# Computational-Genomics-BSC/GenomeAnonymizer

Measured on AMD Instinct MI355X. Metric: reads/sec + bases/sec anonymized, 150 bp paired BAM, 1/2/4/8 MI355X, higher is better.
Workload: dtype u8

## Files before the change

genomeanonymizer_amd/csrc/ganon_batch.h:

```cpp
#ifndef GANON_BATCH_H
#define GANON_BATCH_H

#include <hip/hip_runtime.h>

#include <cstdint>
#include <vector>

#include "../../include/ganon.h"
#include "ganon_ctx.h"

namespace ganon_dev {

constexpr int kBlock = 256;
constexpr int kWaves = kBlock / 64;
constexpr int kTile = 16384;

enum { kSkipClassify = 1, kSkipChunks = 2, kSkipCopy = 4, kSkipCounts = 8 };
constexpr int kGrpRec = 5;
constexpr int kGrpObs = 512;
constexpr int kGrpMaxScopes = 256;
constexpr int kGrpMaxSpan = 1 << 20;
constexpr int64_t kPartAlign = 128;
constexpr int kSegMaxLen = (1 << 14) - 1;
constexpr uint32_t kSegMine = 1u << 31;
// ... 174 lines not shown
  ganon_ref *own_ref = nullptr;
  ganon_dev::DBuf b_ref_start, b_read_len, b_seq_off, b_cig_off, b_n_cig, b_dataset, b_write_scope, b_seq, b_cigar,
      b_incid_off, b_incid_read, b_span_start, b_span_len, b_ref_off, b_keep_pos, b_keep_code;
  ganon_dev::DBuf b_part;
  ganon_dev::DBuf b_long;
  ganon_dev::DBuf b_nseg, b_scost, b_scan_tmp, b_slots, b_slot0;
  ganon_dev::DBuf b_wspart;
  ganon_dev::DBuf b_order;
  int64_t max_scope_incid = 0;
  bool ordered = false;
  ganon_dev::DBuf b_read_end, b_cursor, b_gs0, b_lo, b_linemap, b_groups, b_seg4, b_grp_part, b_far, b_gokey, b_gopay, b_gtkey, b_gtflag, b_out,
      b_scope_calls, b_scope_bases, b_small;
  uint8_t *out = nullptr;
  int32_t *scope_calls = nullptr, *scope_bases = nullptr;
  unsigned long long *totals = nullptr, *static_totals = nullptr, *acc = nullptr, *far_count = nullptr;
  int32_t *rare_tiles = nullptr;
  int32_t *status = nullptr;
  unsigned int *long_count = nullptr;
  unsigned long long *far_need = nullptr;
  size_t flags_bytes = 0;
  ganon_dev::PrepErr *err = nullptr;
  unsigned long long *plan_info = nullptr;
  unsigned long long *paths = nullptr;
  unsigned long long *gated = nullptr;
  unsigned long long *cursor = nullptr;
  ganon_dev::GrpAux *aux = nullptr;
  int32_t n_groups = 0, group_target = 512;
  bool spec = false, spec_ready = false;
  bool spec_sized = false;
  int64_t spec_sizes[4] = {-1, -1, -1, -1};
  bool long_mode = false;
  bool flat_mode = false;
  bool fused = false;
  ganon_dev::DBuf b_desc, b_cand, b_sdirty;
  ganon_dev::DBuf b_xrec, b_xlist, b_xcnt, b_xidx;
  int64_t xcap = 0;
  unsigned int *xcount = nullptr;
  ganon_dev::DBuf b_inc4, b_rbase, b_rrec;
  int64_t n_rrec = 0, n_long_seg = 0;
  unsigned long long *cand = nullptr;
  int64_t *scost = nullptr;
  int64_t n_seg = 0, region = 0, far_cap = 0, n_written = 0, region_per_incid = 0, n_id_ops = 0;
  int64_t max_len = 0, max_seg = 0;
  int64_t far_cap_alloc = 0;
  std::vector<unsigned long long> cursor_h;
  ganon_dev::GrpAux aux_h{};
  unsigned long long static_h[GANON_N_TOTALS] = {0};
  std::vector<void *> huge_allocs;
  ganon_dev::Tile *tiles_h = nullptr;
  int32_t *large_incid = nullptr, *large_written_h = nullptr, *large_ids = nullptr;
  int64_t *tab_off = nullptr;
  uint16_t *tn_tab = nullptr;
  int64_t tn_entries = 0;
  int32_t n_tiles_h = 0, n_large_written_h = 0, n_huge_scopes = 0;
  int32_t *rare_tile_list = nullptr;
  bool ran = false;
};

namespace ganon_prep {

int plan(ganon_ctx *ctx, ganon_dbatch *db, bool allow_spec);
int run(ganon_ctx *ctx, ganon_dbatch *db);
int ws_diag(ganon_ctx *ctx, ganon_dbatch *db);
int batch_error(ganon_ctx *ctx, ganon_dbatch *db);
int grow(ganon_ctx *ctx, ganon_dev::DBuf &b, size_t bytes);
template <typename T>
inline int grow_n(ganon_ctx *ctx, ganon_dev::DBuf &b, size_t count, T **out) {
  int rc = grow(ctx, b, count * sizeof(T));
  *out = static_cast<T *>(b.p);
  return rc;
}

}
// ... 21 lines not shown
```

genomeanonymizer_amd/csrc/ganon_hip.hip:

```cpp
#include <hip/hip_runtime.h>
#include <map>
#include <mutex>

#include <algorithm>
#include <cstdarg>
#include <cstdio>
#include <cstring>
#include <numeric>
#include <string>
#include <type_traits>
#include <vector>

#include "../../include/ganon.h"
#include "ganon_batch.h"
#include "ganon_ctx.h"

using namespace ganon_dev;

namespace {

__global__ void __launch_bounds__(kBlock) k_ref2(const uint8_t *__restrict__ ref, int64_t n_words,
                                                 uint32_t *__restrict__ ref2) {
  for (int64_t w = blockIdx.x * (int64_t)kBlock + threadIdx.x; w < n_words; w += (int64_t)gridDim.x * kBlock) {
    const uint64_t v = load16(ref, 16 * w);
// ... 91 lines not shown
    atomicMax(far_need, n_far_all);
  }
}
}

using ganon_detail::check_launch;
using ganon_detail::fail;
using ganon_detail::KernelScope;

namespace {

constexpr int64_t kFarMaxEntries = int64_t(1) << 30;

void free_buf(DBuf &b) {
  if (b.p) hipFree(b.p);
  b = DBuf{};
}

void free_ref(ganon_ref *r) {
  if (!r) return;
  if (r->nt16) hipFree(r->nt16);
  if (r->ref2) hipFree(r->ref2);
  if (r->bad) hipFree(r->bad);
  delete r;
}

void free_batch(ganon_dbatch *db) {
  DBuf *bufs[] = {&db->b_ref_start, &db->b_read_len, &db->b_seq_off, &db->b_cig_off, &db->b_n_cig, &db->b_dataset,
                  &db->b_write_scope, &db->b_seq, &db->b_cigar, &db->b_incid_off, &db->b_incid_read,
                  &db->b_span_start, &db->b_span_len, &db->b_ref_off, &db->b_keep_pos, &db->b_keep_code,
                  &db->b_read_end, &db->b_wspart, &db->b_cursor, &db->b_gs0, &db->b_lo, &db->b_linemap, &db->b_groups,
                  &db->b_seg4, &db->b_grp_part, &db->b_far, &db->b_gokey, &db->b_gopay, &db->b_gtkey, &db->b_gtflag,
                  &db->b_out, &db->b_scope_calls, &db->b_scope_bases, &db->b_small, &db->b_part, &db->b_long, &db->b_nseg,
                  &db->b_scost, &db->b_scan_tmp, &db->b_slots, &db->b_slot0, &db->b_order, &db->b_desc, &db->b_cand,
                  &db->b_sdirty, &db->b_inc4, &db->b_rbase, &db->b_rrec, &db->b_xrec, &db->b_xlist, &db->b_xcnt, &db->b_xidx};
  for (DBuf *b : bufs) free_buf(*b);
  ganon_huge::release(db);
  free_ref(db->own_ref);
  db->own_ref = nullptr;
}

template <typename T>
int h2d(ganon_ctx *ctx, DBuf &b, const T *src, size_t count, const T **field) {
  T *p = nullptr;
  int rc = ganon_prep::grow_n(ctx, b, count, &p);
  if (rc) return rc;
  if (count) {
    hipError_t e = hipMemcpyAsync(p, src, count * sizeof(T), hipMemcpyHostToDevice, ctx->stream);
    if (e != hipSuccess) return fail(ctx, GANON_E_DEVICE, "hipMemcpyAsync H2D failed: %s", hipGetErrorString(e));
  }
  *field = p;
  return GANON_OK;
}

int ref_create(ganon_ctx *ctx, const uint8_t *nt16, int64_t bytes, ganon_ref **out) {
  *out = nullptr;
  if (bytes < 0 || (bytes > 0 && !nt16)) return fail(ctx, GANON_E_ARG, "bad reference buffer");
  if (2 * bytes >= (int64_t(1) << 40)) return fail(ctx, GANON_E_ARG, "reference over 2^40 bases");
  ganon_ref *r = new ganon_ref();
  r->bytes = bytes;
  r->n_blk = (bytes + 31) / 32;
  const int64_t n_words = (2 * bytes + 15) / 16;
  const int64_t n_bad = (r->n_blk + 63) / 64 + 1;
  hipError_t e = hipMalloc(reinterpret_cast<void **>(&r->nt16), (size_t)bytes + 128);
  if (e == hipSuccess) e = hipMalloc(reinterpret_cast<void **>(&r->ref2), (size_t)(n_words + 2) * 4 + 128);
  if (e == hipSuccess) e = hipMalloc(reinterpret_cast<void **>(&r->bad), (size_t)n_bad * 8 + 128);
  if (e != hipSuccess) {
// ... 767 lines not shown
```

genomeanonymizer_amd/csrc/ganon_prep.hip:

```cpp
#include <hip/hip_runtime.h>

#include <algorithm>
#include <cstring>
#include <type_traits>

#include <rocprim/device/device_scan.hpp>


#include "ganon_batch.h"

using namespace ganon_dev;
using ganon_detail::check_launch;
using ganon_detail::fail;
using ganon_detail::KernelScope;

namespace {

constexpr int kPrepThreads = 256;
constexpr unsigned long long kNone = ~0ull;
constexpr int kCursors = 256;
constexpr int64_t kFarMax = int64_t(1) << 28;

struct Raw {
  const int32_t *ref_start, *read_len, *n_cig, *write_scope;
// ... 33 lines not shown
  return cost ? cost[s] / target : (incid_off[s] + weight * s) / target;
}

enum { kPartWritten = 0, kPartMaxLen, kPartMaxSeg, kPartIdOps, kPartHuge, kPartWsHash, kParts };

__device__ __forceinline__ unsigned long long block_sum_u64(unsigned long long v, unsigned long long *ws) {
  for (int o = 32; o > 0; o >>= 1) {
    const uint32_t lo = __shfl_xor((uint32_t)v, o), hi = __shfl_xor((uint32_t)(v >> 32), o);
    v += ((unsigned long long)hi << 32) | lo;
  }
  __syncthreads();
  if ((threadIdx.x & 63) == 0) ws[threadIdx.x >> 6] = v;
  __syncthreads();
  unsigned long long t = 0;
  for (int w = 0; w < kWaves; ++w) t += ws[w];
  return t;
}
#ifndef GANON_SCAN_U
#define GANON_SCAN_U 4
#endif
constexpr int kScanReadsPerBlock = GANON_SCAN_U * kPrepThreads;
constexpr int kScanScopesPerBlock = 4 * kPrepThreads;

struct ScanOut {
  int32_t *read_end;
  int32_t *long_list;
  unsigned int *long_count;
  longlong2 *gmeta;
  int64_t g_bound;
  unsigned long long *part;
  int64_t part_stride;
  int32_t *nseg;
  int4 *desc;
  unsigned long long *cand;
  int32_t *xidx;
  int4 *xrec;
  unsigned int *xcount;
  uint32_t xper;
};


__device__ __forceinline__ unsigned long long shfl64(unsigned long long v, int lane) {
  const uint32_t lo = __shfl((uint32_t)v, lane), hi = __shfl((uint32_t)(v >> 32), lane);
  return ((unsigned long long)hi << 32) | lo;
}

__device__ __forceinline__ void scan_candidate(unsigned long long *__restrict__ cand, long long key, int64_t so) {
  const unsigned long long v = ~(unsigned long long)so;
  const int lane = threadIdx.x & 63;
  unsigned long long pending = __ballot(key >= 0);
  while (pending) {
    const int leader = __ffsll((long long)pending) - 1;
    const uint32_t klo = __builtin_amdgcn_readlane((uint32_t)key, leader),
                   khi = __builtin_amdgcn_readlane((uint32_t)((unsigned long long)key >> 32), leader);
    const long long lk = (long long)(((unsigned long long)khi << 32) | klo);
    const bool same = key == lk;
    unsigned long long x = same ? v : 0ull;
#pragma unroll
    for (int o = 32; o > 0; o >>= 1) {
      const unsigned long long y = shfl64(x, lane ^ o);
      x = y > x ? y : x;
    }
    if (lane == leader) atomicMax(&cand[lk], x);
    pending &= ~__ballot(same);
  }
}

__device__ __forceinline__ void block_parts(unsigned long long (&acc)[kParts], unsigned long long *__restrict__ part,
                                            int64_t stride) {
  __shared__ unsigned long long ws[kWaves][kParts];
  const int lane = threadIdx.x & 63, wave = threadIdx.x >> 6;
#pragma unroll
  for (int k = 0; k < kParts; ++k) {
    unsigned long long v = acc[k];
#pragma unroll
    for (int o = 32; o > 0; o >>= 1) {
      const unsigned long long x = shfl64(v, lane ^ o);
      v = (k == kPartMaxLen || k == kPartMaxSeg) ? (x > v ? x : v) : v + x;
    }
    if (lane == 0) ws[wave][k] = v;
  }
  __syncthreads();
  if (threadIdx.x < kParts) {
    const int k = threadIdx.x;
    unsigned long long v = 0;
    for (int w = 0; w < kWaves; ++w)
      v = (k == kPartMaxLen || k == kPartMaxSeg) ? (ws[w][k] > v ? ws[w][k] : v) : v + ws[w][k];
    part[stride * k + blockIdx.x] = v;
  }
}

struct CigarWalk {
  long long rl;
  int ns, nid, bad_op;
};

__device__ __forceinline__ CigarWalk wave_cigar_walk(const uint32_t *__restrict__ cg, int nc, int L) {
  const int lane = threadIdx.x & 63;
// ... 55 lines not shown
    int L[kScanU], nc[kScanU], rs[kScanU], ws[kScanU], ds[kScanU];
    Off co[kScanU], so[kScanU];
    bool ok[kScanU];
    {
      int64_t co64[kScanU], so64[kScanU];
#pragma unroll
      for (int u = 0; u < kScanU; ++u) {
        const int64_t r = r0 + tid + kPrepThreads * u;
        ok[u] = r < r1;
        const int64_t rr = ok[u] ? r : r0;
        L[u] = R.read_len[rr];
        nc[u] = R.n_cig[rr];
        co64[u] = R.cig_off[rr];
        rs[u] = R.ref_start[rr];
        so64[u] = R.seq_off[rr];
        ws[u] = R.write_scope[rr];
        ds[u] = R.dataset[rr];
      }
#pragma unroll
      for (int u = 0; u < kScanU; ++u) {
        const int64_t r = r0 + tid + kPrepThreads * u;
        if (ok[u]) {
          if (L[u] < 0 || so64[u] < 0 || so64[u] + ((int64_t)L[u] + 1) / 2 > R.seq_bytes) { report(err, kErrReadSeq, r); ok[u] = false; }
          else if (nc[u] < 0 || co64[u] < 0 || co64[u] + nc[u] > R.n_cigar_ops) { report(err, kErrReadCigar, r); ok[u] = false; }
          if (ds[u] > 1) report(err, kErrReadDataset, r);
          if (ws[u] < -1 || ws[u] >= R.n_scopes) { report(err, kErrReadWriteScope, r, ws[u]); ok[u] = false; }
          if (L[u] >= (1 << 24)) report(err, kErrReadLong, r);
        }
        co[u] = ok[u] ? (Off)co64[u] : (Off)0;
        so[u] = ok[u] ? (Off)so64[u] : (Off)0;
      }
    }
    uint32_t w0[kScanU];
    int wo[kScanU];
#pragma unroll
    for (int u = 0; u < kScanU; ++u) {
      w0[u] = ok[u] && nc[u] > 0 ? R.cigar[co[u]] : 0u;
      wo[u] = O.cand && ok[u] && ws[u] >= 0 && L[u] > 0 ? (int)R.incid_off[ws[u]] : -1;
    }
    if (O.cand) {
#pragma unroll
      for (int u = 0; u < kScanU; ++u) {
        long long key = -1;
        if (wo[u] >= 0) {
          const uint64_t x = (uint64_t)wo[u] + (uint64_t)weight * (uint64_t)ws[u];
          int64_t g = x >> 32 ? (int64_t)(x / (uint64_t)target) : (int64_t)((uint32_t)x / (uint32_t)target);
          g = g < 0 ? 0 : (g > O.g_bound - 1 ? O.g_bound - 1 : g);
          key = 2 * g + (ds[u] & 1);
        }
        scan_candidate(O.cand, key, (int64_t)so[u]);
      }
    }
#pragma unroll
    for (int u = 0; u < kScanU; ++u) {
      const int64_t r = r0 + tid + kPrepThreads * u;
      if (ok[u]) {
        n_wr += ws[u] >= 0;
        if (ws[u] >= 0) hsum += ws_hash((int)r);
        mx_len = max(mx_len, (uint32_t)L[u]);
        if (nc[u] > kScanLongCigar) {
          O.long_list[atomicAdd(O.long_count, 1u)] = (int32_t)r;
          continue;
        }
        int64_t rl = 0;
        int q = 0, ns = 0, nid = 0;
        int fq = 0, fn = 0;
        int fp = 0;
        bool good = true;
        for (int k = 0; k < nc[u]; ++k) {
          const uint32_t w = k == 0 ? w0[u] : R.cigar[co[u] + k];
          const int op = (int)(w & 0xF);
          const int len = (int)(w >> 4);
          if (op > 8) { report(err, kErrCigarOp, r, op); good = false; break; }
          if (is_aligned_op(op)) {
            if (q < L[u]) {
              if (ns == 0) {
                fq = q;
                fp = (int)rl;
                fn = min(min(len, L[u] - q), kSegMaxLen);
              }
              ns += (min(len, L[u] - q) + kSegMaxLen - 1) / kSegMaxLen;
            }
            q += len;
            rl += len;
          } else if (op == 1 || op == 4) {
// ... 388 lines not shown

__global__ void __launch_bounds__(kPrepThreads) k_prep_pieces(const unsigned long long *__restrict__ lo, int n_cand,
                                                              LineMap M, int64_t seq_bytes, int4 *__restrict__ groups,
                                                              const unsigned long long *__restrict__ gate) {
  if (gate) {
    if (gate[7]) return;
    n_cand = (int)min((unsigned long long)n_cand, 2 * gate[5]);
  }
  for (int64_t c = blockIdx.x * (int64_t)kPrepThreads + threadIdx.x; c < n_cand; c += (int64_t)gridDim.x * kPrepThreads) {
    const unsigned long long k = lo[c];
    int4 pc = piece(0, 0);
    if (k != kNone) {
      const int64_t line = (int64_t)(k >> 7);
      unsigned long long win = 0;
      for (unsigned h = hash_line(line, M.hsize);; h = (h + 1) & (unsigned)(M.hsize - 1))
        if (M.hkey[h] == (unsigned long long)line + 1) {
          win = M.hval[h];
          break;
        }
      if ((win & ((1ull << 25) - 1)) == (unsigned long long)c) {
        const int64_t next = map_next(M, line);
        const int64_t a = map_any_below(M, line) ? line * kPartAlign : 0;
        pc = piece(a, next < 0 ? seq_bytes : next * kPartAlign);
      }
    } else if (c == 0) {
      bool any = false;
      for (int64_t w = 0; w < M.n2 && !any; ++w) any = M.l2[w] != 0;
      if (!any) pc = piece(0, seq_bytes);
    }
    groups[kGrpRec * (c >> 1) + 2 + 2 * (c & 1)] = pc;
  }
}

__global__ void __launch_bounds__(kPrepThreads) k_prep_cands(const Raw R, const longlong2 *__restrict__ gmeta,
                                                             int n_groups, long long region_per_incid,
                                                             const unsigned long long *__restrict__ cand,
                                                             unsigned long long *__restrict__ lo, int4 *__restrict__ groups,
                                                             LineMap M, unsigned long long *__restrict__ ws_part,
                                                             const unsigned long long *__restrict__ gate,
                                                             uint8_t *__restrict__ sdirty, const uint64_t *__restrict__ bad,
                                                             int64_t n_blk) {
  const int64_t g = blockIdx.x * (int64_t)kPrepThreads + threadIdx.x;
  if (gate[7]) return;
  if (g < R.n_scopes) {
    const int64_t sl = R.span_len[g], ro = R.ref_off[g];
    sdirty[g] = sl > 0 && sl <= kGrpMaxSpan && !ref_clean(bad, n_blk, ro, (int)sl);
  }
  if (g >= n_groups) return;
  if ((unsigned long long)g >= gate[5]) {
    ws_part[g] = 0;
    return;
  }
  const longlong2 m0 = gmeta[g];
  const longlong2 m1 = (unsigned long long)g + 1 < gate[5] ? gmeta[g + 1] : make_longlong2(R.n_scopes, R.n_incid);
  const int s0 = (int)m0.x, s1 = (int)m1.x;
  const int64_t i0 = m0.y, i1 = m1.y;
  const int64_t region = i0 * region_per_incid + (int64_t)kGrpObs * g;
  const int cap = (int)min((i1 - i0) * region_per_incid + kGrpObs, (long long)(INT32_MAX / 2));
  groups[kGrpRec * g] = make_int4(s0, s1, (int)(uint32_t)i0, (int)(uint32_t)((uint64_t)i0 >> 32));
  groups[kGrpRec * g + 1] = make_int4((int)(uint32_t)i1, (int)(uint32_t)((uint64_t)i1 >> 32), (int)(uint32_t)i1,
                                      (int)(uint32_t)((uint64_t)i1 >> 32));
  groups[kGrpRec * g + 3] = make_int4((int)(uint32_t)region, (int)(uint32_t)((uint64_t)region >> 32), cap, 0);
#pragma unroll
  for (int d = 0; d < 2; ++d) {
    const unsigned long long c = cand[2 * g + d];
    const unsigned long long k = c ? ~c : kNone;
    lo[2 * g + d] = k;
    if (k != kNone) map_mark(M, k, (uint32_t)(2 * g + d));
  }
}

__device__ __forceinline__ void block_scan2(int a, int b, int &ea, int &eb, int &ta, int &tb, int *ws) {
  const int lane = threadIdx.x & 63, wave = threadIdx.x >> 6;
  int ia = a, ib = b;
#pragma unroll
  for (int o = 1; o < 64; o <<= 1) {
    const int xa = __shfl_up(ia, o), xb = __shfl_up(ib, o);
    if (lane >= o) {
      ia += xa;
      ib += xb;
    }
  }
  if (lane == 63) {
    ws[wave] = ia;
    ws[kWaves + wave] = ib;
  }
  __syncthreads();
  int ba = 0, bb = 0;
  ta = tb = 0;
#pragma unroll
  for (int w = 0; w < kWaves; ++w) {
    const int va = ws[w], vb = ws[kWaves + w];
    if (w < wave) {
      ba += va;
      bb += vb;
    }
    ta += va;
    tb += vb;
  }
  ea = ba + ia - a;
  eb = bb + ib - b;
  __syncthreads();
// ... 791 lines not shown
    return rc;
  db->B.read_end = read_end;
  db->ran = false;
  const Raw R = raw_of(db);
  const int tgt0 = ctx->group_target ? ctx->group_target : 704;
  const long long w0 = weight_of(tgt0);
  const int64_t g_bound = ns ? (db->n_incid + w0 * (ns - 1)) / tgt0 + 1 : 1;
  const bool want_fused = ctx->fused_flat && (ctx->prep_long == -1 || ctx->prep_long == 2);
  const bool same = db->spec_ready && db->spec_sizes[0] == nr && db->spec_sizes[1] == ns &&
                    db->spec_sizes[2] == db->n_incid && db->spec_sizes[3] == tgt0 && db->flat_mode &&
                    ctx->last_plan == db && db->fused == want_fused;
  ctx->last_plan = db;
  const bool sized = !same && ctx->spec_shape_ok && ctx->spec_tgt == tgt0 && ctx->prep_long == -1;
  const bool spec = allow_spec && ctx->spec_plan && (same || sized);
  db->spec = spec;
  db->spec_sized = spec && sized;
  if (!spec) {
    db->n_groups = 0;
    db->spec_ready = false;
  }
  db->fused = want_fused;
  const int64_t spec_rpi = !spec ? 0 : db->spec_sized ? ctx->spec_rpi : db->region_per_incid;
  longlong2 *gm = nullptr;
  unsigned long long *part = nullptr;
  const int64_t rb = (nr + kScanReadsPerBlock - 1) / kScanReadsPerBlock;
  const int64_t sb = (ns + kScanScopesPerBlock - 1) / kScanScopesPerBlock;
  const int64_t nb = std::max<int64_t>(1, rb + sb);
  if (nb > INT32_MAX) return fail(ctx, GANON_E_ARG, "batch too large");
  int32_t *long_list = nullptr;
  if ((rc = grow_n(ctx, db->b_gs0, (size_t)g_bound, &gm)) ||
      (rc = grow_n(ctx, db->b_part, (size_t)kParts * (nb + kLongGrid), &part)) ||
      (rc = grow_n(ctx, db->b_long, (size_t)std::max<int64_t>(nr, 1), &long_list)))
    return rc;
  unsigned long long *cand = nullptr;
  int4 *desc = nullptr, *xrec = nullptr;
  int2 *xlist = nullptr;
  int32_t *xidx = nullptr;
  uint8_t *sdirty = nullptr;
  if (db->fused) {
    const int64_t xwant = std::min<int64_t>(
        INT32_MAX, ctx->xrec_init > 0 && db->xcap == 0 ? (int64_t)ctx->xrec_init
                                                       : std::max<int64_t>({db->xcap, int64_t(65536), nr / 8}));
    if ((rc = grow_n(ctx, db->b_desc, (size_t)std::max<int64_t>(nr, 1), &desc)) ||
        (rc = grow_n(ctx, db->b_cand, 2 * (size_t)g_bound, &cand)) ||
        (rc = grow_n(ctx, db->b_sdirty, (size_t)std::max<int64_t>(ns, 1), &sdirty)) ||
        (rc = grow_n(ctx, db->b_xrec, (size_t)xwant, &xrec)) ||
        (rc = grow_n(ctx, db->b_xlist, (size_t)std::max<int64_t>(db->n_incid, 1), &xlist)) ||
        (rc = grow_n(ctx, db->b_xidx, (size_t)std::max<int64_t>(nr, 1), &xidx)))
      return rc;
    db->xcap = std::min<int64_t>(INT32_MAX, (int64_t)((db->b_xrec.bytes - 128) / sizeof(int4)));
    if (ctx->xrec_init > 0 && db->xcap > xwant) db->xcap = xwant;
  }
  db->cand = cand;
  unsigned int *long_count = db->long_count;
  const int64_t pstride = nb + kLongGrid;
  if ((rc = grow_n(ctx, db->b_xcnt, (size_t)kXStripes * kXStride, &db->xcount))) return rc;
  const ScanOut O{read_end, long_list, long_count, gm, g_bound, part, pstride, nullptr, desc, cand, xidx, xrec, db->xcount,
                  (uint32_t)(xrec ? db->xcap / kXStripes : 0)};
  const int spec_maxseg = db->fused ? kFusedMaxSeg : 1;
  {
    KernelScope ks(ctx, "prep_scan");
    HIP_OR_FAIL(hipMemsetAsync(db->err, 0, db->flags_bytes, st));
    HIP_OR_FAIL(hipMemsetAsync(db->xcount, 0, (size_t)kXStripes * kXStride * sizeof(unsigned int), st));
    if (cand) HIP_OR_FAIL(hipMemsetAsync(cand, 0, 2 * (size_t)g_bound * sizeof *cand, st));
    const bool narrow = db->seq_bytes < INT32_MAX && db->n_cigar_ops < INT32_MAX;
    hipLaunchKernelGGL(narrow ? k_prep_scan<true> : k_prep_scan<false>, dim3((unsigned)nb), dim3(kPrepThreads), 0, st, R,
                       db->err, O, w0, (long long)tgt0, (int)rb);
    hipLaunchKernelGGL(k_prep_reduce, dim3(1), dim3(kReduceThreads), 0, st, R, part, pstride, (int)nb, w0, (long long)tgt0,
                       g_bound, db->plan_info, static_cast<const PrepErr *>(db->err),
                       (long long)spec_rpi, static_cast<const unsigned int *>(long_count), spec_maxseg,
                       static_cast<const unsigned int *>(db->xcount), (unsigned int)O.xper);
    if ((rc = check_launch(ctx, "k_prep_scan"))) return rc;
  }
  if (spec && !db->spec_sized) return GANON_OK;
  if (spec) {
    db->long_mode = false;
    db->flat_mode = true;
    db->region_per_incid = spec_rpi;
    db->group_target = tgt0;
    db->n_id_ops = 0;
    db->max_len = 48 * spec_rpi;
    db->max_seg = spec_maxseg;
    db->n_huge_scopes = 0;
    db->n_written = -1;
    db->scost = nullptr;
    return size_plan(ctx, db, ns ? g_bound : 0, tgt0, R);
  }
  unsigned long long info[6] = {0, 0, 0, 0, 0, 0};
  PrepErr e{};
  unsigned int n_long = 0;
  std::vector<unsigned int> xc((size_t)kXStripes * kXStride, 0u);
  HIP_OR_FAIL(ganon_detail::readback(info, db->plan_info, sizeof info, st));
  HIP_OR_FAIL(ganon_detail::readback(&e, db->err, sizeof e, st));
  HIP_OR_FAIL(ganon_detail::readback(&n_long, long_count, sizeof n_long, st));
  if (db->fused)
    HIP_OR_FAIL(ganon_detail::readback(xc.data(), db->xcount, xc.size() * sizeof(unsigned int), st));
  HIP_OR_FAIL(ganon_detail::sync_stream(st));
  if (!e.code && n_long) {
    KernelScope ks(ctx, "prep_scan_long");
    const unsigned gl = (unsigned)std::min<int64_t>(kLongGrid, ((int64_t)n_long + 3) / 4);
    ScanOut OL = O;
    OL.part = part + nb;
    if ((rc = grow_n(ctx, db->b_nseg, (size_t)std::max<int64_t>(nr, 1), &OL.nseg))) return rc;
    hipLaunchKernelGGL(k_prep_scan_long, dim3(gl), dim3(kPrepThreads), 0, st, R, db->err, OL, (int)n_long);
    hipLaunchKernelGGL(k_prep_reduce, dim3(1), dim3(kReduceThreads), 0, st, R, part, pstride, (int)(nb + gl), w0,
                       (long long)tgt0, g_bound, db->plan_info, static_cast<const PrepErr *>(db->err), 0ll,
                       static_cast<const unsigned int *>(long_count), spec_maxseg,
                       static_cast<const unsigned int *>(db->xcount), (unsigned int)O.xper);
    if ((rc = check_launch(ctx, "k_prep_scan_long"))) return rc;
    HIP_OR_FAIL(ganon_detail::readback(info, db->plan_info, sizeof info, st));
    HIP_OR_FAIL(ganon_detail::readback(&e, db->err, sizeof e, st));
    HIP_OR_FAIL(ganon_detail::sync_stream(st));
  }
  if (e.code) return fail(ctx, GANON_E_ARG, err_text(e.code), e.index, e.a, e.b);
  const unsigned long long max_len = info[3], max_seg = info[4];
  db->long_mode = ctx->prep_long == 1 || (ctx->prep_long == -1 && max_seg > 1 && max_len > kLongReadLen);
  const bool fused_multi = db->fused && n_long == 0 && max_seg <= (unsigned long long)kFusedMaxSeg;
  int64_t xfull = 0;
  for (int k = 0; k < kXStripes; ++k) xfull = std::max<int64_t>(xfull, xc[(size_t)kXStride * k]);
  if (fused_multi && max_seg > 1 && !db->long_mode && xfull > db->xcap / kXStripes) {
    int4 *x = nullptr;
    const int64_t want = std::min<int64_t>(INT32_MAX, kXStripes * (xfull + xfull / 4 + 64));
    if (kXStripes * xfull >= INT32_MAX) return fail(ctx, GANON_E_ARG, "batch too large: %lld extras records per stripe", (long long)xfull);
    if ((rc = grow_n(ctx, db->b_xrec, (size_t)want, &x))) return rc;
    db->xcap = want;
    return plan(ctx, db, false);
  }
  db->flat_mode = !db->long_mode && (max_seg <= 1 || fused_multi) && (ctx->prep_long == -1 || ctx->prep_long == 2);
  db->fused = db->fused && db->flat_mode && n_long == 0;
  if (!db->fused) db->cand = nullptr;
  db->region_per_incid = (int64_t)((max_len + 47) / 48);
  db->group_target = ctx->group_target ? ctx->group_target : db->long_mode ? 2816 : 704;
  db->n_id_ops = (int64_t)info[0];
  db->max_len = (int64_t)max_len;
  db->max_seg = (int64_t)max_seg;
  db->n_huge_scopes = (int32_t)info[1];
  db->n_written = (int64_t)info[2];
  if ((double)db->n_incid * (double)db->region_per_incid > 4e9)
    return fail(ctx, GANON_E_ARG, "batch too large: %lld incidences of reads up to %llu bases (split it)",
                (long long)db->n_incid, max_len);
  const long long w = weight_of(db->group_target);
  int64_t ng = ns ? (int64_t)info[5] : 0;
  db->scost = nullptr;
  if (db->long_mode && ns) {
    if ((rc = grow_n(ctx, db->b_nseg, (size_t)std::max<int64_t>(nr, 1), &nseg))) return rc;
    if (nr) hipLaunchKernelGGL(k_prep_nseg, dim3(grid_for(nr)), dim3(kPrepThreads), 0, st, R, nseg);
    int64_t *cost = nullptr;
    if ((rc = grow_n(ctx, db->b_scost, (size_t)ns + 1, &cost))) return rc;
    hipLaunchKernelGGL(k_prep_scope_cost, dim3(grid_for(ns + 1)), dim3(kPrepThreads), 0, st, R, nseg, w, cost);
    if ((rc = check_launch(ctx, "k_prep_scope_cost"))) return rc;
    int64_t *rbase = nullptr;
    if ((rc = grow_n(ctx, db->b_rbase, (size_t)std::max<int64_t>(nr, 1), &rbase))) return rc;
    size_t tb = 0, tb2 = 0;
    HIP_OR_FAIL(rocprim::exclusive_scan(nullptr, tb, cost, cost, (int64_t)0, (size_t)ns + 1, rocprim::plus<int64_t>(), st));
    if (nr) HIP_OR_FAIL(rocprim::exclusive_scan(nullptr, tb2, nseg, rbase, (int64_t)0, (size_t)nr, rocprim::plus<int64_t>(), st));
    tb = std::max(tb, tb2);
    void *tmp = nullptr;
    if ((rc = grow_n(ctx, db->b_scan_tmp, tb, reinterpret_cast<uint8_t **>(&tmp)))) return rc;
    HIP_OR_FAIL(rocprim::exclusive_scan(tmp, tb, cost, cost, (int64_t)0, (size_t)ns + 1, rocprim::plus<int64_t>(), st));
    int64_t last[2] = {0, 0}, rb_last = 0;
    int32_t ns_last = 0;
    HIP_OR_FAIL(ganon_detail::readback(last, cost + ns - 1, sizeof last, st));
    if (nr) {
      HIP_OR_FAIL(rocprim::exclusive_scan(tmp, tb, nseg, rbase, (int64_t)0, (size_t)nr, rocprim::plus<int64_t>(), st));
      HIP_OR_FAIL(ganon_detail::readback(&rb_last, rbase + nr - 1, sizeof rb_last, st));
      HIP_OR_FAIL(ganon_detail::readback(&ns_last, nseg + nr - 1, sizeof ns_last, st));
    }
    HIP_OR_FAIL(ganon_detail::sync_stream(st));
    db->scost = cost;
    ng = last[0] / db->group_target + 1;
    db->n_rrec = rb_last + ns_last;
    db->n_long_seg = last[1] - w * ns;
    int4 *i4 = nullptr, *rr = nullptr;
    uint8_t *sd = nullptr;
    if ((rc = grow_n(ctx, db->b_inc4, (size_t)std::max<int64_t>(db->n_incid, 1), &i4)) ||
        (rc = grow_n(ctx, db->b_rrec, (size_t)std::max<int64_t>(db->n_rrec, 1), &rr)) ||
        (rc = grow_n(ctx, db->b_sdirty, (size_t)ns, &sd)))
      return rc;
  } else if (ns && db->group_target != tgt0) {
    return fail(ctx, GANON_E_STATE, "group target changed during the plan");
  }
  if (db->flat_mode && ns) ng = g_bound;
  return size_plan(ctx, db, ng, tgt0, R);
}

int run(ganon_ctx *ctx, ganon_dbatch *db) {
  const Raw R = raw_of(db);
  int rc;
  if (!db->n_groups) return GANON_OK;
  if (db->flat_mode) {
    {
      KernelScope ks(ctx, "prep_emit");
      HIP_OR_FAIL(hipMemsetAsync(db->b_linemap.p, 0, (size_t)line_map_words(db) * 8, ctx->stream));
    }
    if (db->fused) {
      KernelScope ks(ctx, "prep_cands");
      hipLaunchKernelGGL(k_prep_cands, dim3(grid_for(std::max<int64_t>(db->n_groups, db->n_scopes), INT32_MAX)),
                         dim3(kPrepThreads), 0, ctx->stream, R, static_cast<const longlong2 *>(db->b_gs0.p), db->n_groups,
                         (long long)db->region_per_incid, static_cast<const unsigned long long *>(db->cand),
                         static_cast<unsigned long long *>(db->b_lo.p), static_cast<int4 *>(db->b_groups.p), line_map(db),
                         static_cast<unsigned long long *>(db->b_wspart.p),
                         static_cast<const unsigned long long *>(db->plan_info), static_cast<uint8_t *>(db->b_sdirty.p),
                         db->ref->bad, db->ref->n_blk);
      if ((rc = check_launch(ctx, "k_prep_cands"))) return rc;
    } else if ((rc = launch_emit(ctx, db, R, 1))) {
      return rc;
    }
  } else if ((rc = launch_groups(ctx, db, R)) || (rc = launch_emit(ctx, db, R, 1))) {
    return rc;
  }
  return launch_pieces(ctx, db);
}

int ws_diag(ganon_ctx *ctx, ganon_dbatch *db) {
  hipLaunchKernelGGL(k_prep_ws_diag, dim3(grid_for(db->n_reads)), dim3(kPrepThreads), 0, ctx->stream, raw_of(db),
                     db->err);
  return check_launch(ctx, "k_prep_ws_diag");
}

int batch_error(ganon_ctx *ctx, ganon_dbatch *db) {
  PrepErr e{};
  HIP_OR_FAIL(ganon_detail::readback(&e, db->err, sizeof e, ctx->stream));
  HIP_OR_FAIL(ganon_detail::sync_stream(ctx->stream));
  if (e.code) return fail(ctx, GANON_E_ARG, err_text(e.code), e.index, e.a, e.b);
  return GANON_OK;
}

}

int ganon_ref_blocks(ganon_ctx *ctx, ganon_ref *ref) {
  if (!ref->n_blk) return GANON_OK;
  const int64_t n_round = (ref->n_blk + 63) & ~(int64_t)63;
  hipLaunchKernelGGL(k_ref_blocks, dim3(grid_for(n_round)), dim3(kPrepThreads), 0, ctx->stream, ref->nt16, ref->bytes,
// ... 4 lines not shown
```

Before: 16.26 billion.

## Compute per-group candidate minima in cands kernel instead of scan atomics

Removes the wave-level ballot/shuffle atomicMax candidate tracking from the prep scan kernel, along with its buffer and memset. The per-group, per-dataset minimum sequence offset is now computed in k_prep_cands: 16 lanes per group walk the group's incidence list with early exit once both parities have a hit, then reduce with shuffles. The goal is to take contended atomics and a serialized ballot loop out of the hot scan path. In exchange, the cands kernel launches 16x more threads and does extra gathered loads per incidence.

New measurement: 16.37 billion, median of 2. Within noise of the previous version (+0.7%).

```diff
diff --git a/genomeanonymizer_amd/csrc/ganon_batch.h b/genomeanonymizer_amd/csrc/ganon_batch.h
--- a/genomeanonymizer_amd/csrc/ganon_batch.h
+++ b/genomeanonymizer_amd/csrc/ganon_batch.h
@@ -230,13 +230,12 @@
   bool long_mode = false;
   bool flat_mode = false;
   bool fused = false;
-  ganon_dev::DBuf b_desc, b_cand, b_sdirty;
+  ganon_dev::DBuf b_desc, b_sdirty;
   ganon_dev::DBuf b_xrec, b_xlist, b_xcnt, b_xidx;
   int64_t xcap = 0;
   unsigned int *xcount = nullptr;
   ganon_dev::DBuf b_inc4, b_rbase, b_rrec;
   int64_t n_rrec = 0, n_long_seg = 0;
-  unsigned long long *cand = nullptr;
   int64_t *scost = nullptr;
   int64_t n_seg = 0, region = 0, far_cap = 0, n_written = 0, region_per_incid = 0, n_id_ops = 0;
   int64_t max_len = 0, max_seg = 0;
diff --git a/genomeanonymizer_amd/csrc/ganon_hip.hip b/genomeanonymizer_amd/csrc/ganon_hip.hip
--- a/genomeanonymizer_amd/csrc/ganon_hip.hip
+++ b/genomeanonymizer_amd/csrc/ganon_hip.hip
@@ -147,7 +147,7 @@
                   &db->b_read_end, &db->b_wspart, &db->b_cursor, &db->b_gs0, &db->b_lo, &db->b_linemap, &db->b_groups,
                   &db->b_seg4, &db->b_grp_part, &db->b_far, &db->b_gokey, &db->b_gopay, &db->b_gtkey, &db->b_gtflag,
                   &db->b_out, &db->b_scope_calls, &db->b_scope_bases, &db->b_small, &db->b_part, &db->b_long, &db->b_nseg,
-                  &db->b_scost, &db->b_scan_tmp, &db->b_slots, &db->b_slot0, &db->b_order, &db->b_desc, &db->b_cand,
+                  &db->b_scost, &db->b_scan_tmp, &db->b_slots, &db->b_slot0, &db->b_order, &db->b_desc,
                   &db->b_sdirty, &db->b_inc4, &db->b_rbase, &db->b_rrec, &db->b_xrec, &db->b_xlist, &db->b_xcnt, &db->b_xidx};
   for (DBuf *b : bufs) free_buf(*b);
   ganon_huge::release(db);
diff --git a/genomeanonymizer_amd/csrc/ganon_prep.hip b/genomeanonymizer_amd/csrc/ganon_prep.hip
--- a/genomeanonymizer_amd/csrc/ganon_prep.hip
+++ b/genomeanonymizer_amd/csrc/ganon_prep.hip
@@ -89,7 +89,6 @@
   int64_t part_stride;
   int32_t *nseg;
   int4 *desc;
-  unsigned long long *cand;
   int32_t *xidx;
   int4 *xrec;
   unsigned int *xcount;
@@ -100,27 +99,6 @@
 __device__ __forceinline__ unsigned long long shfl64(unsigned long long v, int lane) {
   const uint32_t lo = __shfl((uint32_t)v, lane), hi = __shfl((uint32_t)(v >> 32), lane);
   return ((unsigned long long)hi << 32) | lo;
-}
-
-__device__ __forceinline__ void scan_candidate(unsigned long long *__restrict__ cand, long long key, int64_t so) {
-  const unsigned long long v = ~(unsigned long long)so;
-  const int lane = threadIdx.x & 63;
-  unsigned long long pending = __ballot(key >= 0);
-  while (pending) {
-    const int leader = __ffsll((long long)pending) - 1;
-    const uint32_t klo = __builtin_amdgcn_readlane((uint32_t)key, leader),
-                   khi = __builtin_amdgcn_readlane((uint32_t)((unsigned long long)key >> 32), leader);
-    const long long lk = (long long)(((unsigned long long)khi << 32) | klo);
-    const bool same = key == lk;
-    unsigned long long x = same ? v : 0ull;
-#pragma unroll
-    for (int o = 32; o > 0; o >>= 1) {
-      const unsigned long long y = shfl64(x, lane ^ o);
-      x = y > x ? y : x;
-    }
-    if (lane == leader) atomicMax(&cand[lk], x);
-    pending &= ~__ballot(same);
-  }
 }
 
 __device__ __forceinline__ void block_parts(unsigned long long (&acc)[kParts], unsigned long long *__restrict__ part,
@@ -242,25 +220,8 @@
       }
     }
     uint32_t w0[kScanU];
-    int wo[kScanU];
-#pragma unroll
-    for (int u = 0; u < kScanU; ++u) {
-      w0[u] = ok[u] && nc[u] > 0 ? R.cigar[co[u]] : 0u;
-      wo[u] = O.cand && ok[u] && ws[u] >= 0 && L[u] > 0 ? (int)R.incid_off[ws[u]] : -1;
-    }
-    if (O.cand) {
-#pragma unroll
-      for (int u = 0; u < kScanU; ++u) {
-        long long key = -1;
-        if (wo[u] >= 0) {
-          const uint64_t x = (uint64_t)wo[u] + (uint64_t)weight * (uint64_t)ws[u];
-          int64_t g = x >> 32 ? (int64_t)(x / (uint64_t)target) : (int64_t)((uint32_t)x / (uint32_t)target);
-          g = g < 0 ? 0 : (g > O.g_bound - 1 ? O.g_bound - 1 : g);
-          key = 2 * g + (ds[u] & 1);
-        }
-        scan_candidate(O.cand, key, (int64_t)so[u]);
-      }
-    }
+#pragma unroll
+    for (int u = 0; u < kScanU; ++u) w0[u] = ok[u] && nc[u] > 0 ? R.cigar[co[u]] : 0u;
 #pragma unroll
     for (int u = 0; u < kScanU; ++u) {
       const int64_t r = r0 + tid + kPrepThreads * u;
@@ -715,41 +676,96 @@
   }
 }
 
+constexpr int kCandRow = 16;
+constexpr int kCandRows = 4;
+
+template <int N>
+__device__ __forceinline__ void cand_rows(const Raw &R, int64_t i, int64_t i1, int s0, int s1, unsigned long long &mn0,
+                                          unsigned long long &mn1) {
+  int r[N], ws[N], L[N], ds[N];
+  int64_t so[N];
+  bool in[N];
+#pragma unroll
+  for (int u = 0; u < N; ++u) {
+    const int64_t k = i + kCandRow * u;
+    r[u] = k < i1 ? R.incid_read[k] : -1;
+  }
+#pragma unroll
+  for (int u = 0; u < N; ++u) {
+    in[u] = r[u] >= 0 && r[u] < R.n_reads;
+    ws[u] = in[u] ? R.write_scope[r[u]] : -1;
+    L[u] = in[u] ? R.read_len[r[u]] : 0;
+    ds[u] = in[u] ? R.dataset[r[u]] : 0;
+    so[u] = in[u] ? R.seq_off[r[u]] : 0;
+  }
+#pragma unroll
+  for (int u = 0; u < N; ++u) {
+    const bool mine = in[u] && ws[u] >= s0 && ws[u] < s1 && L[u] > 0;
+    const unsigned long long v = (unsigned long long)so[u];
+    const unsigned long long v0 = mine && !(ds[u] & 1) ? v : kNone, v1 = mine && (ds[u] & 1) ? v : kNone;
+    mn0 = v0 < mn0 ? v0 : mn0;
+    mn1 = v1 < mn1 ? v1 : mn1;
+  }
+}
+
 __global__ void __launch_bounds__(kPrepThreads) k_prep_cands(const Raw R, const longlong2 *__restrict__ gmeta,
                                                              int n_groups, long long region_per_incid,
-                                                             const unsigned long long *__restrict__ cand,
                                                              unsigned long long *__restrict__ lo, int4 *__restrict__ groups,
                                                              LineMap M, unsigned long long *__restrict__ ws_part,
                                                              const unsigned long long *__restrict__ gate,
                                                              uint8_t *__restrict__ sdirty, const uint64_t *__restrict__ bad,
                                                              int64_t n_blk) {
-  const int64_t g = blockIdx.x * (int64_t)kPrepThreads + threadIdx.x;
+  static_assert(kCandRow == 16 && kPrepThreads % kCandRow == 0, "a row is a quarter of a wave");
+  const int64_t t = blockIdx.x * (int64_t)kPrepThreads + threadIdx.x;
   if (gate[7]) return;
-  if (g < R.n_scopes) {
-    const int64_t sl = R.span_len[g], ro = R.ref_off[g];
-    sdirty[g] = sl > 0 && sl <= kGrpMaxSpan && !ref_clean(bad, n_blk, ro, (int)sl);
-  }
+  if (t < R.n_scopes) {
+    const int64_t sl = R.span_len[t], ro = R.ref_off[t];
+    sdirty[t] = sl > 0 && sl <= kGrpMaxSpan && !ref_clean(bad, n_blk, ro, (int)sl);
+  }
+  const int64_t g = t / kCandRow;
+  const int sub = threadIdx.x & (kCandRow - 1);
   if (g >= n_groups) return;
   if ((unsigned long long)g >= gate[5]) {
-    ws_part[g] = 0;
+    if (sub == 0) ws_part[g] = 0;
     return;
   }
   const longlong2 m0 = gmeta[g];
   const longlong2 m1 = (unsigned long long)g + 1 < gate[5] ? gmeta[g + 1] : make_longlong2(R.n_scopes, R.n_incid);
   const int s0 = (int)m0.x, s1 = (int)m1.x;
   const int64_t i0 = m0.y, i1 = m1.y;
-  const int64_t region = i0 * region_per_incid + (int64_t)kGrpObs * g;
-  const int cap = (int)min((i1 - i0) * region_per_incid + kGrpObs, (long long)(INT32_MAX / 2));
-  groups[kGrpRec * g] = make_int4(s0, s1, (int)(uint32_t)i0, (int)(uint32_t)((uint64_t)i0 >> 32));
-  groups[kGrpRec * g + 1] = make_int4((int)(uint32_t)i1, (int)(uint32_t)((uint64_t)i1 >> 32), (int)(uint32_t)i1,
-                                      (int)(uint32_t)((uint64_t)i1 >> 32));
-  groups[kGrpRec * g + 3] = make_int4((int)(uint32_t)region, (int)(uint32_t)((uint64_t)region >> 32), cap, 0);
-#pragma unroll
-  for (int d = 0; d < 2; ++d) {
-    const unsigned long long c = cand[2 * g + d];
-    const unsigned long long k = c ? ~c : kNone;
-    lo[2 * g + d] = k;
-    if (k != kNone) map_mark(M, k, (uint32_t)(2 * g + d));
+  if (sub == 0) {
+    const int64_t region = i0 * region_per_incid + (int64_t)kGrpObs * g;
+    const int cap = (int)min((i1 - i0) * region_per_incid + kGrpObs, (long long)(INT32_MAX / 2));
+    groups[kGrpRec * g] = make_int4(s0, s1, (int)(uint32_t)i0, (int)(uint32_t)((uint64_t)i0 >> 32));
+    groups[kGrpRec * g + 1] = make_int4((int)(uint32_t)i1, (int)(uint32_t)((uint64_t)i1 >> 32), (int)(uint32_t)i1,
+                                        (int)(uint32_t)((uint64_t)i1 >> 32));
+    groups[kGrpRec * g + 3] = make_int4((int)(uint32_t)region, (int)(uint32_t)((uint64_t)region >> 32), cap, 0);
+  }
+  unsigned long long mn0 = kNone, mn1 = kNone;
+  const int row_shift = threadIdx.x & 63 & ~(kCandRow - 1);
+  int64_t i = i0 + sub;
+  cand_rows<1>(R, i, i1, s0, s1, mn0, mn1);
+  i += kCandRow;
+  for (;;) {
+    const unsigned f0 = (unsigned)(__ballot(mn0 != kNone) >> row_shift) & 0xFFFFu;
+    const unsigned f1 = (unsigned)(__ballot(mn1 != kNone) >> row_shift) & 0xFFFFu;
+    if ((f0 && f1) || i - sub >= i1) break;
+    cand_rows<kCandRows>(R, i, i1, s0, s1, mn0, mn1);
+    i += kCandRow * kCandRows;
+  }
+#pragma unroll
+  for (int o = kCandRow / 2; o > 0; o >>= 1) {
+    const unsigned long long x0 = ((unsigned long long)(uint32_t)__shfl_xor((int)(mn0 >> 32), o, kCandRow) << 32) |
+                                  (uint32_t)__shfl_xor((int)(uint32_t)mn0, o, kCandRow);
+    const unsigned long long x1 = ((unsigned long long)(uint32_t)__shfl_xor((int)(mn1 >> 32), o, kCandRow) << 32) |
+                                  (uint32_t)__shfl_xor((int)(uint32_t)mn1, o, kCandRow);
+    mn0 = x0 < mn0 ? x0 : mn0;
+    mn1 = x1 < mn1 ? x1 : mn1;
+  }
+  if (sub < 2) {
+    const unsigned long long k = sub ? mn1 : mn0;
+    lo[2 * g + sub] = k;
+    if (k != kNone) map_mark(M, k, (uint32_t)(2 * g + sub));
   }
 }
 
@@ -1608,7 +1624,6 @@
       (rc = grow_n(ctx, db->b_part, (size_t)kParts * (nb + kLongGrid), &part)) ||
       (rc = grow_n(ctx, db->b_long, (size_t)std::max<int64_t>(nr, 1), &long_list)))
     return rc;
-  unsigned long long *cand = nullptr;
   int4 *desc = nullptr, *xrec = nullptr;
   int2 *xlist = nullptr;
   int32_t *xidx = nullptr;
@@ -1618,7 +1633,6 @@
         INT32_MAX, ctx->xrec_init > 0 && db->xcap == 0 ? (int64_t)ctx->xrec_init
                                                        : std::max<int64_t>({db->xcap, int64_t(65536), nr / 8}));
     if ((rc = grow_n(ctx, db->b_desc, (size_t)std::max<int64_t>(nr, 1), &desc)) ||
-        (rc = grow_n(ctx, db->b_cand, 2 * (size_t)g_bound, &cand)) ||
         (rc = grow_n(ctx, db->b_sdirty, (size_t)std::max<int64_t>(ns, 1), &sdirty)) ||
         (rc = grow_n(ctx, db->b_xrec, (size_t)xwant, &xrec)) ||
         (rc = grow_n(ctx, db->b_xlist, (size_t)std::max<int64_t>(db->n_incid, 1), &xlist)) ||
@@ -1627,18 +1641,16 @@
     db->xcap = std::min<int64_t>(INT32_MAX, (int64_t)((db->b_xrec.bytes - 128) / sizeof(int4)));
     if (ctx->xrec_init > 0 && db->xcap > xwant) db->xcap = xwant;
   }
-  db->cand = cand;
   unsigned int *long_count = db->long_count;
   const int64_t pstride = nb + kLongGrid;
   if ((rc = grow_n(ctx, db->b_xcnt, (size_t)kXStripes * kXStride, &db->xcount))) return rc;
-  const ScanOut O{read_end, long_list, long_count, gm, g_bound, part, pstride, nullptr, desc, cand, xidx, xrec, db->xcount,
+  const ScanOut O{read_end, long_list, long_count, gm, g_bound, part, pstride, nullptr, desc, xidx, xrec, db->xcount,
                   (uint32_t)(xrec ? db->xcap / kXStripes : 0)};
   const int spec_maxseg = db->fused ? kFusedMaxSeg : 1;
   {
     KernelScope ks(ctx, "prep_scan");
     HIP_OR_FAIL(hipMemsetAsync(db->err, 0, db->flags_bytes, st));
     HIP_OR_FAIL(hipMemsetAsync(db->xcount, 0, (size_t)kXStripes * kXStride * sizeof(unsigned int), st));
-    if (cand) HIP_OR_FAIL(hipMemsetAsync(cand, 0, 2 * (size_t)g_bound * sizeof *cand, st));
     const bool narrow = db->seq_bytes < INT32_MAX && db->n_cigar_ops < INT32_MAX;
     hipLaunchKernelGGL(narrow ? k_prep_scan<true> : k_prep_scan<false>, dim3((unsigned)nb), dim3(kPrepThreads), 0, st, R,
                        db->err, O, w0, (long long)tgt0, (int)rb);
@@ -1704,7 +1716,6 @@
   }
   db->flat_mode = !db->long_mode && (max_seg <= 1 || fused_multi) && (ctx->prep_long == -1 || ctx->prep_long == 2);
   db->fused = db->fused && db->flat_mode && n_long == 0;
-  if (!db->fused) db->cand = nullptr;
   db->region_per_incid = (int64_t)((max_len + 47) / 48);
   db->group_target = ctx->group_target ? ctx->group_target : db->long_mode ? 2816 : 704;
   db->n_id_ops = (int64_t)info[0];
@@ -1771,10 +1782,10 @@
     }
     if (db->fused) {
       KernelScope ks(ctx, "prep_cands");
-      hipLaunchKernelGGL(k_prep_cands, dim3(grid_for(std::max<int64_t>(db->n_groups, db->n_scopes), INT32_MAX)),
+      hipLaunchKernelGGL(k_prep_cands,
+                         dim3(grid_for(std::max<int64_t>((int64_t)kCandRow * db->n_groups, db->n_scopes), INT32_MAX)),
                          dim3(kPrepThreads), 0, ctx->stream, R, static_cast<const longlong2 *>(db->b_gs0.p), db->n_groups,
-                         (long long)db->region_per_incid, static_cast<const unsigned long long *>(db->cand),
-                         static_cast<unsigned long long *>(db->b_lo.p), static_cast<int4 *>(db->b_groups.p), line_map(db),
+                         (long long)db->region_per_incid, static_cast<unsigned long long *>(db->b_lo.p), static_cast<int4 *>(db->b_groups.p), line_map(db),
                          static_cast<unsigned long long *>(db->b_wspart.p),
                          static_cast<const unsigned long long *>(db->plan_info), static_cast<uint8_t *>(db->b_sdirty.p),
                          db->ref->bad, db->ref->n_blk);
```

## Compute per-group min sequence offset in cands kernel instead of scan atomics

Applied to the files above, without the earlier changes.

Removes the per-read candidate atomicMax reduction from the prep scan kernel, along with its cand buffer and the memset that cleared it. Instead, k_prep_cands assigns one wave per group, walks the group's incidences (up to a few 64-wide trips), and takes a wave-level min of seq offsets per dataset parity. The aim is to cut atomic contention and extra memory traffic in the scan. In exchange the cands launch grows 64x in threads. The bounded trip count with early exit may also change results when a group's first 256 incidences lack a candidate, and membership is now derived from incidence ranges rather than the scan's group formula.

Result: no change. 16.02 billion before, 15.94 billion after (-0.5%).

```diff
diff --git a/genomeanonymizer_amd/csrc/ganon_batch.h b/genomeanonymizer_amd/csrc/ganon_batch.h
--- a/genomeanonymizer_amd/csrc/ganon_batch.h
+++ b/genomeanonymizer_amd/csrc/ganon_batch.h
@@ -230,13 +230,12 @@
   bool long_mode = false;
   bool flat_mode = false;
   bool fused = false;
-  ganon_dev::DBuf b_desc, b_cand, b_sdirty;
+  ganon_dev::DBuf b_desc, b_sdirty;
   ganon_dev::DBuf b_xrec, b_xlist, b_xcnt, b_xidx;
   int64_t xcap = 0;
   unsigned int *xcount = nullptr;
   ganon_dev::DBuf b_inc4, b_rbase, b_rrec;
   int64_t n_rrec = 0, n_long_seg = 0;
-  unsigned long long *cand = nullptr;
   int64_t *scost = nullptr;
   int64_t n_seg = 0, region = 0, far_cap = 0, n_written = 0, region_per_incid = 0, n_id_ops = 0;
   int64_t max_len = 0, max_seg = 0;
diff --git a/genomeanonymizer_amd/csrc/ganon_hip.hip b/genomeanonymizer_amd/csrc/ganon_hip.hip
--- a/genomeanonymizer_amd/csrc/ganon_hip.hip
+++ b/genomeanonymizer_amd/csrc/ganon_hip.hip
@@ -147,7 +147,7 @@
                   &db->b_read_end, &db->b_wspart, &db->b_cursor, &db->b_gs0, &db->b_lo, &db->b_linemap, &db->b_groups,
                   &db->b_seg4, &db->b_grp_part, &db->b_far, &db->b_gokey, &db->b_gopay, &db->b_gtkey, &db->b_gtflag,
                   &db->b_out, &db->b_scope_calls, &db->b_scope_bases, &db->b_small, &db->b_part, &db->b_long, &db->b_nseg,
-                  &db->b_scost, &db->b_scan_tmp, &db->b_slots, &db->b_slot0, &db->b_order, &db->b_desc, &db->b_cand,
+                  &db->b_scost, &db->b_scan_tmp, &db->b_slots, &db->b_slot0, &db->b_order, &db->b_desc,
                   &db->b_sdirty, &db->b_inc4, &db->b_rbase, &db->b_rrec, &db->b_xrec, &db->b_xlist, &db->b_xcnt, &db->b_xidx};
   for (DBuf *b : bufs) free_buf(*b);
   ganon_huge::release(db);
diff --git a/genomeanonymizer_amd/csrc/ganon_prep.hip b/genomeanonymizer_amd/csrc/ganon_prep.hip
--- a/genomeanonymizer_amd/csrc/ganon_prep.hip
+++ b/genomeanonymizer_amd/csrc/ganon_prep.hip
@@ -89,7 +89,6 @@
   int64_t part_stride;
   int32_t *nseg;
   int4 *desc;
-  unsigned long long *cand;
   int32_t *xidx;
   int4 *xrec;
   unsigned int *xcount;
@@ -100,27 +99,6 @@
 __device__ __forceinline__ unsigned long long shfl64(unsigned long long v, int lane) {
   const uint32_t lo = __shfl((uint32_t)v, lane), hi = __shfl((uint32_t)(v >> 32), lane);
   return ((unsigned long long)hi << 32) | lo;
-}
-
-__device__ __forceinline__ void scan_candidate(unsigned long long *__restrict__ cand, long long key, int64_t so) {
-  const unsigned long long v = ~(unsigned long long)so;
-  const int lane = threadIdx.x & 63;
-  unsigned long long pending = __ballot(key >= 0);
-  while (pending) {
-    const int leader = __ffsll((long long)pending) - 1;
-    const uint32_t klo = __builtin_amdgcn_readlane((uint32_t)key, leader),
-                   khi = __builtin_amdgcn_readlane((uint32_t)((unsigned long long)key >> 32), leader);
-    const long long lk = (long long)(((unsigned long long)khi << 32) | klo);
-    const bool same = key == lk;
-    unsigned long long x = same ? v : 0ull;
-#pragma unroll
-    for (int o = 32; o > 0; o >>= 1) {
-      const unsigned long long y = shfl64(x, lane ^ o);
-      x = y > x ? y : x;
-    }
-    if (lane == leader) atomicMax(&cand[lk], x);
-    pending &= ~__ballot(same);
-  }
 }
 
 __device__ __forceinline__ void block_parts(unsigned long long (&acc)[kParts], unsigned long long *__restrict__ part,
@@ -242,25 +220,8 @@
       }
     }
     uint32_t w0[kScanU];
-    int wo[kScanU];
-#pragma unroll
-    for (int u = 0; u < kScanU; ++u) {
-      w0[u] = ok[u] && nc[u] > 0 ? R.cigar[co[u]] : 0u;
-      wo[u] = O.cand && ok[u] && ws[u] >= 0 && L[u] > 0 ? (int)R.incid_off[ws[u]] : -1;
-    }
-    if (O.cand) {
-#pragma unroll
-      for (int u = 0; u < kScanU; ++u) {
-        long long key = -1;
-        if (wo[u] >= 0) {
-          const uint64_t x = (uint64_t)wo[u] + (uint64_t)weight * (uint64_t)ws[u];
-          int64_t g = x >> 32 ? (int64_t)(x / (uint64_t)target) : (int64_t)((uint32_t)x / (uint32_t)target);
-          g = g < 0 ? 0 : (g > O.g_bound - 1 ? O.g_bound - 1 : g);
-          key = 2 * g + (ds[u] & 1);
-        }
-        scan_candidate(O.cand, key, (int64_t)so[u]);
-      }
-    }
+#pragma unroll
+    for (int u = 0; u < kScanU; ++u) w0[u] = ok[u] && nc[u] > 0 ? R.cigar[co[u]] : 0u;
 #pragma unroll
     for (int u = 0; u < kScanU; ++u) {
       const int64_t r = r0 + tid + kPrepThreads * u;
@@ -715,9 +676,20 @@
   }
 }
 
+constexpr int kCandTrips = 4;
+
+__device__ __forceinline__ unsigned long long wave_min_u64(unsigned long long v) {
+  const int lane = threadIdx.x & 63;
+#pragma unroll
+  for (int o = 32; o > 0; o >>= 1) {
+    const unsigned long long y = shfl64(v, lane ^ o);
+    v = y < v ? y : v;
+  }
+  return v;
+}
+
 __global__ void __launch_bounds__(kPrepThreads) k_prep_cands(const Raw R, const longlong2 *__restrict__ gmeta,
                                                              int n_groups, long long region_per_incid,
-                                                             const unsigned long long *__restrict__ cand,
                                                              unsigned long long *__restrict__ lo, int4 *__restrict__ groups,
                                                              LineMap M, unsigned long long *__restrict__ ws_part,
                                                              const unsigned long long *__restrict__ gate,
@@ -725,6 +697,40 @@
                                                              int64_t n_blk) {
   const int64_t g = blockIdx.x * (int64_t)kPrepThreads + threadIdx.x;
   if (gate[7]) return;
+  const int64_t wg = g >> 6;
+  if (wg < n_groups && (unsigned long long)wg < gate[5]) {
+    const int lane = threadIdx.x & 63;
+    const longlong2 m0 = gmeta[wg];
+    const longlong2 m1 = (unsigned long long)wg + 1 < gate[5] ? gmeta[wg + 1] : make_longlong2(R.n_scopes, R.n_incid);
+    const int s0 = (int)m0.x, s1 = (int)m1.x;
+    const int64_t i0 = m0.y, i1 = m1.y;
+    unsigned long long mn0 = kNone, mn1 = kNone;
+    for (int trip = 0; trip < kCandTrips; ++trip) {
+      const int64_t i = i0 + 64 * trip + lane;
+      unsigned long long v0 = kNone, v1 = kNone;
+      if (i < i1) {
+        const int r = R.incid_read[i];
+        if (r >= 0 && r < R.n_reads) {
+          const int ws = R.write_scope[r], L = R.read_len[r], d = R.dataset[r];
+          const unsigned long long so = (unsigned long long)R.seq_off[r];
+          if (ws >= s0 && ws < s1 && L > 0 && R.incid_off[ws] <= i && i < R.incid_off[ws + 1]) {
+            v0 = d & 1 ? kNone : so;
+            v1 = d & 1 ? so : kNone;
+          }
+        }
+      }
+      const unsigned long long w0 = wave_min_u64(v0), w1 = wave_min_u64(v1);
+      mn0 = w0 < mn0 ? w0 : mn0;
+      mn1 = w1 < mn1 ? w1 : mn1;
+      if ((mn0 != kNone && mn1 != kNone) || i0 + 64 * (trip + 1) >= i1) break;
+    }
+    if (lane == 0) {
+      lo[2 * wg] = mn0;
+      lo[2 * wg + 1] = mn1;
+      if (mn0 != kNone) map_mark(M, mn0, (uint32_t)(2 * wg));
+      if (mn1 != kNone) map_mark(M, mn1, (uint32_t)(2 * wg + 1));
+    }
+  }
   if (g < R.n_scopes) {
     const int64_t sl = R.span_len[g], ro = R.ref_off[g];
     sdirty[g] = sl > 0 && sl <= kGrpMaxSpan && !ref_clean(bad, n_blk, ro, (int)sl);
@@ -744,13 +750,6 @@
   groups[kGrpRec * g + 1] = make_int4((int)(uint32_t)i1, (int)(uint32_t)((uint64_t)i1 >> 32), (int)(uint32_t)i1,
                                       (int)(uint32_t)((uint64_t)i1 >> 32));
   groups[kGrpRec * g + 3] = make_int4((int)(uint32_t)region, (int)(uint32_t)((uint64_t)region >> 32), cap, 0);
-#pragma unroll
-  for (int d = 0; d < 2; ++d) {
-    const unsigned long long c = cand[2 * g + d];
-    const unsigned long long k = c ? ~c : kNone;
-    lo[2 * g + d] = k;
-    if (k != kNone) map_mark(M, k, (uint32_t)(2 * g + d));
-  }
 }
 
 __device__ __forceinline__ void block_scan2(int a, int b, int &ea, int &eb, int &ta, int &tb, int *ws) {
@@ -1608,7 +1607,6 @@
       (rc = grow_n(ctx, db->b_part, (size_t)kParts * (nb + kLongGrid), &part)) ||
       (rc = grow_n(ctx, db->b_long, (size_t)std::max<int64_t>(nr, 1), &long_list)))
     return rc;
-  unsigned long long *cand = nullptr;
   int4 *desc = nullptr, *xrec = nullptr;
   int2 *xlist = nullptr;
   int32_t *xidx = nullptr;
@@ -1618,7 +1616,6 @@
         INT32_MAX, ctx->xrec_init > 0 && db->xcap == 0 ? (int64_t)ctx->xrec_init
                                                        : std::max<int64_t>({db->xcap, int64_t(65536), nr / 8}));
     if ((rc = grow_n(ctx, db->b_desc, (size_t)std::max<int64_t>(nr, 1), &desc)) ||
-        (rc = grow_n(ctx, db->b_cand, 2 * (size_t)g_bound, &cand)) ||
         (rc = grow_n(ctx, db->b_sdirty, (size_t)std::max<int64_t>(ns, 1), &sdirty)) ||
         (rc = grow_n(ctx, db->b_xrec, (size_t)xwant, &xrec)) ||
         (rc = grow_n(ctx, db->b_xlist, (size_t)std::max<int64_t>(db->n_incid, 1), &xlist)) ||
@@ -1627,18 +1624,16 @@
     db->xcap = std::min<int64_t>(INT32_MAX, (int64_t)((db->b_xrec.bytes - 128) / sizeof(int4)));
     if (ctx->xrec_init > 0 && db->xcap > xwant) db->xcap = xwant;
   }
-  db->cand = cand;
   unsigned int *long_count = db->long_count;
   const int64_t pstride = nb + kLongGrid;
   if ((rc = grow_n(ctx, db->b_xcnt, (size_t)kXStripes * kXStride, &db->xcount))) return rc;
-  const ScanOut O{read_end, long_list, long_count, gm, g_bound, part, pstride, nullptr, desc, cand, xidx, xrec, db->xcount,
+  const ScanOut O{read_end, long_list, long_count, gm, g_bound, part, pstride, nullptr, desc, xidx, xrec, db->xcount,
                   (uint32_t)(xrec ? db->xcap / kXStripes : 0)};
   const int spec_maxseg = db->fused ? kFusedMaxSeg : 1;
   {
     KernelScope ks(ctx, "prep_scan");
     HIP_OR_FAIL(hipMemsetAsync(db->err, 0, db->flags_bytes, st));
     HIP_OR_FAIL(hipMemsetAsync(db->xcount, 0, (size_t)kXStripes * kXStride * sizeof(unsigned int), st));
-    if (cand) HIP_OR_FAIL(hipMemsetAsync(cand, 0, 2 * (size_t)g_bound * sizeof *cand, st));
     const bool narrow = db->seq_bytes < INT32_MAX && db->n_cigar_ops < INT32_MAX;
     hipLaunchKernelGGL(narrow ? k_prep_scan<true> : k_prep_scan<false>, dim3((unsigned)nb), dim3(kPrepThreads), 0, st, R,
                        db->err, O, w0, (long long)tgt0, (int)rb);
@@ -1704,7 +1699,6 @@
   }
   db->flat_mode = !db->long_mode && (max_seg <= 1 || fused_multi) && (ctx->prep_long == -1 || ctx->prep_long == 2);
   db->fused = db->fused && db->flat_mode && n_long == 0;
-  if (!db->fused) db->cand = nullptr;
   db->region_per_incid = (int64_t)((max_len + 47) / 48);
   db->group_target = ctx->group_target ? ctx->group_target : db->long_mode ? 2816 : 704;
   db->n_id_ops = (int64_t)info[0];
@@ -1771,10 +1765,9 @@
     }
     if (db->fused) {
       KernelScope ks(ctx, "prep_cands");
-      hipLaunchKernelGGL(k_prep_cands, dim3(grid_for(std::max<int64_t>(db->n_groups, db->n_scopes), INT32_MAX)),
+      hipLaunchKernelGGL(k_prep_cands, dim3(grid_for(std::max<int64_t>(64 * (int64_t)db->n_groups, db->n_scopes), INT32_MAX)),
                          dim3(kPrepThreads), 0, ctx->stream, R, static_cast<const longlong2 *>(db->b_gs0.p), db->n_groups,
-                         (long long)db->region_per_incid, static_cast<const unsigned long long *>(db->cand),
-                         static_cast<unsigned long long *>(db->b_lo.p), static_cast<int4 *>(db->b_groups.p), line_map(db),
+                         (long long)db->region_per_incid, static_cast<unsigned long long *>(db->b_lo.p), static_cast<int4 *>(db->b_groups.p), line_map(db),
                          static_cast<unsigned long long *>(db->b_wspart.p),
                          static_cast<const unsigned long long *>(db->plan_info), static_cast<uint8_t *>(db->b_sdirty.p),
                          db->ref->bad, db->ref->n_blk);
```
